# ragoragino/partitionedhashjoin

Measured on AMD Instinct MI355X. Metric: probe+build tuples/sec at 10M⋈200M; achieved HBM GB/s vs roofline, 1/2/4/8 GPU, higher is better.
Workload: dtype int64

## Files before the change

### partitionedhashjoin_amd/csrc/phj_capi.hip

```cpp
#include <hip/hip_runtime.h>

#include <algorithm>
#include <atomic>
#include <cmath>
#include <cstdio>
#include <cstdlib>
#include <cstring>
#include <exception>
#include <functional>
#include <string>
#include <type_traits>
#include <unordered_map>
#include <vector>

#ifndef PHJ_PREAGG
#define PHJ_PREAGG 1
#endif
#ifndef PHJ_HOT_EARLY_R
#define PHJ_HOT_EARLY_R 1
#endif
#ifndef PHJ_HOT_FREE_CUS
#define PHJ_HOT_FREE_CUS 6
#endif
#ifndef PHJ_COL_LOAD16
#define PHJ_COL_LOAD16 0
#endif
#ifndef PHJ_P1_PROF
#define PHJ_P1_PROF 0
#endif
#ifndef PHJ_CL_PROF
#define PHJ_CL_PROF 0
#endif

#include "../../include/phj.h"
#include "phj_cluster.h"
#include "phj_join.h"
#include "phj_inner.h"
#include "phj_outer.h"
#include "phj_index.h"
#include "phj_ordinal.h"
#include "phj_agg.h"
#include "phj_mat.h"
#include "phj_partition.h"
#include "phj_hot.h"
#include "phj_table.h"
#include "phj_member.h"
#include "phj_lookup.h"

using namespace phj;

namespace {

constexpr double kNPDefaultRatio = 2.0;
constexpr uint32_t kNPRegionBuckets = 1024;
constexpr int kOnePassMax = 256;
// ... 126 lines not shown
    DevBuf mat_mark, mat_cnt, mat_rows;
    DevBuf row_hit, row_only, row_cnt;
    DevBuf agg_acc, agg_cnt, agg_rows, agg_res;
    uint64_t agg_n = 0;
    uint64_t mat_n = 0;
    uint64_t idx_n = 0;
    DevBuf gather_bad;
    std::vector<hipEvent_t> evpool;
    size_t evnext = 0;
    std::vector<TimerRec> timers;
    std::string err;
    Tuning tune;
    bool last_fused = false;
    bool dry = false;
    hipEvent_t last_ev = nullptr;
    hipStream_t last_ev_stream = nullptr;
    uint32_t since_ev = 0;
    unsigned long long* count_host = nullptr;
    unsigned long long* count_pin = nullptr;
    unsigned long long* count_pin_dev = nullptr;
    DevBuf cl_done;
    bool count_pin_failed = false, count_pinned = false;
    unsigned long long* split_words = nullptr;
    bool defer_timers = false;
    bool lean_timers = false;
    bool timer_skipped = false;
    void* p1_clear = nullptr;
    size_t p1_clear_bytes = 0;
    void* p1_cleared = nullptr;
    void* s_zeroed = nullptr;
    size_t s_zeroed_bytes = 0;
    void* s_zero_pending = nullptr;
    size_t s_zero_pending_bytes = 0;
    int poison = -1;
    DevBuf hot;
    void* hot_clean = nullptr;
    uint32_t hot_clean_nb = 0;
    int hot_mode = 0;
    bool hot_on = false, hot_ran = false;
    uint64_t hot_n = 0;
    uint32_t hot_min_mass = 0;
    hipEvent_t hot_fork = nullptr, hot_join = nullptr;
    uint32_t p1_free_cus = 0;
    bool p1_cols = false;
    std::vector<phj_index*> indexes;
};

struct phj_index {
    phj_ctx* owner = nullptr;
    IxBucket* tab = nullptr;
    size_t bytes = 0;
    NPHome g{};
    int hk = 0;
    uint64_t seed = 0;
    uint64_t rows = 0, distinct = 0;
    uint32_t max_wgs = 1;
    uint32_t flags = 0;
    int64_t* first_rows = nullptr;
    uint32_t acc_wgs = 1;
};

namespace {

int set_err(phj_ctx* c, int code, const std::string& msg) {
    if (c) c->err = msg;
    return code;
}

#define PHJ_HIP(ctx, expr)                                                                   \
    do {                                                                                     \
        hipError_t e_ = (expr);                                                              \
        if (e_ != hipSuccess)                                                                \
            return set_err(ctx, PHJ_ERR_HIP,                                                 \
                           std::string(#expr) + ": " + hipGetErrorString(e_));               \
    } while (0)

#define PHJ_LAUNCHED(ctx, what)                                                              \
    do {                                                                                     \
        (ctx)->since_ev++;                                                                   \
        hipError_t e_ = hipGetLastError();                                                   \
        if (e_ != hipSuccess)                                                                \
            return set_err(ctx, PHJ_ERR_HIP, std::string("launch ") + what + ": " +         \
                                                 hipGetErrorString(e_));                     \
    } while (0)

#define PHJ_TRY(expr)           \
    do {                        \
        int rc_ = (expr);       \
        if (rc_ != PHJ_OK) return rc_; \
    } while (0)

int ensure(phj_ctx* c, DevBuf& b, size_t bytes) {
    if (bytes == 0) bytes = 16;
    if (b.bytes >= bytes) return PHJ_OK;
    if (b.p) {
        PHJ_HIP(c, hipStreamSynchronize(c->stream));
        PHJ_HIP(c, hipStreamSynchronize(c->aux));
        PHJ_HIP(c, hipFree(b.p));
        b.p = nullptr;
        b.bytes = 0;
    }
    const size_t rounded = (bytes + 4095) & ~size_t(4095);
    hipError_t e = hipMalloc(&b.p, rounded);
    if (e != hipSuccess) {
        b.p = nullptr;
        return set_err(c, PHJ_ERR_NOMEM, "hipMalloc(" + std::to_string(rounded) + "): " + hipGetErrorString(e));
    }
    b.bytes = rounded;
    if (c->poison >= 0) {
        PHJ_HIP(c, hipMemsetAsync(b.p, c->poison, rounded, c->stream));
        PHJ_HIP(c, hipStreamSynchronize(c->stream));
    }
    return PHJ_OK;
}

void free_buf(DevBuf& b) {
    if (b.p) (void)hipFree(b.p);
    b.p = nullptr;
    b.bytes = 0;
}

hipEvent_t new_event() {
    hipEvent_t e = nullptr;
    const unsigned tries[3] = {hipEventDisableSystemFence, hipEventReleaseToDevice, hipEventDefault};
    for (unsigned f : tries) {
        if (hipEventCreateWithFlags(&e, f) == hipSuccess) break;
        (void)hipGetLastError();
        e = nullptr;
    }
    return e;
// ... 340 lines not shown
        size_t l;
        bool operator==(const Key& o) const { return f == o.f && b == o.b && l == o.l; }
    };
    struct Hash {
        size_t operator()(const Key& k) const {
            return std::hash<const void*>()(k.f) ^ (static_cast<size_t>(k.b) << 20) ^ (k.l * 0x9E3779B97F4A7C15ull);
        }
    };
    thread_local std::unordered_map<Key, int, Hash> cache;
    const Key k{kfn, block, lds};
    auto it = cache.find(k);
    if (it != cache.end()) return it->second;
    int occ = 0;
    if (hipOccupancyMaxActiveBlocksPerMultiprocessor(&occ, kfn, block, lds) != hipSuccess) {
        (void)hipGetLastError();
        occ = 0;
    }
    cache.emplace(k, occ);
    return occ;
}

template <int BLOCK, int ITEMS, bool IN_AOS, bool OUT_AOS, int ROWS = 0>
int launch_pass_t(phj_ctx* c, int hk, const PassArgs& a, uint32_t grid, const std::string& prefix,
                  uint64_t n, uint32_t hist_len) {
    static_assert(ROWS == 0 || IN_AOS, "row numbers are synthesised by pass 1");
    if (ROWS != 0 && a.keys_only) return set_err(c, PHJ_ERR_INVALID, "row-number pass 1: no keys-only form");
    constexpr uint64_t kcol = ROWS == 1 ? 8 : 0;
    constexpr int T = BLOCK * ITEMS;
    constexpr int NW = BLOCK / 64;
    const size_t hist_lds = static_cast<size_t>(NW) * a.nbins * 4;
    const size_t sc_lds = scatter_lds_bytes(T, a.nbins, NW, a.chunk_cursor != nullptr);
    const std::string hname = prefix + ".hist", cname = prefix + ".scan", sname = prefix + ".scatter";
    if (a.chunk_cursor) {
        const bool zeroed = a.chunk_cursor == c->s_zeroed && chunk_state_bytes(a.nbins) <= c->s_zeroed_bytes;
        if (a.chunk_cursor == c->s_zeroed) c->s_zeroed = nullptr;
        if (a.chunk_cursor == c->p1_cleared) c->p1_cleared = nullptr;
        else if (!zeroed) PHJ_HIP(c, hipMemsetAsync(a.chunk_cursor, 0, chunk_state_bytes(a.nbins), c->ks));
        c->since_ev++;
        const uint64_t sbytes = n * (a.keys_only ? 24 : 32) - (c->p1_cols ? n * 8 : 0) - n * kcol + (a.out_dig ? n * (a.dig_wide ? 2 : 1) : 0);
        PHJ_TRY(timer_begin(c, sname.c_str(), sbytes));
        if constexpr (IN_AOS && OUT_AOS && ITEMS <= 8) {
            const uint32_t ntiles = static_cast<uint32_t>((n + T - 1) / T);
            const uint32_t per = (ntiles + a.nshards - 1) / a.nshards;
            const bool pipe = a.keys_only && c->tune.p1_pipe && BLOCK == 512 && ITEMS == 8;
            const bool is_r = prefix.rfind("R.", 0) == 0;
            const bool hot = a.hot_code != nullptr;
            const size_t lds = pipe ? chunk_pipe_lds_bytes(T, a.nbins) + chunk_pipe_hot_lds_bytes(a.nbins, hot ? 1 : 0)
                               : a.keys_only ? chunk_codes_lds_bytes(T, a.nbins) : sc_lds;
            const void* kfn = nullptr;
            int kblock = BLOCK;
            bool cols_form = false;
            if (a.keys_only && pipe) {
                if constexpr (BLOCK == 512 && ITEMS == 8) {
                    const int dpt = a.nbins > 2 * BLOCK ? 4 : a.nbins > BLOCK ? 2 : 1;
                    if (c->tune.p1_block == 1024) {
                        kblock = 1024;
                        const int kpf = is_r ? 1 : 2;
                        if (hot && dpt == 4) return set_err(c, PHJ_ERR_STATE, "hot-key pre-aggregation: more digits than threads");
                        if (c->p1_cols && dpt == 4) return set_err(c, PHJ_ERR_STATE, "key column: more digits than threads");
                        const int cols = !c->p1_cols ? 0 : PHJ_COL_LOAD16 != 0 && n >= 2 ? 2 : 1;
                        cols_form = cols != 0;
                        kfn = with_hash(hk, [&](auto h) {
                            constexpr int HK = decltype(h)::value;
                            return dpt == 4 ? pipe1024<HK, 2>(kpf) : pipe1024<HK, 1>(kpf, hot, cols);
                        });
                    } else if (hot) {
                        return set_err(c, PHJ_ERR_STATE, "hot-key pre-aggregation needs the 1024-thread code pass");
                    } else
                        kfn = with_hash(hk, [&](auto h) {
                            constexpr int HK = decltype(h)::value;
                            return dpt == 4 ? reinterpret_cast<const void*>(&k_chunk_codes_pipe<BLOCK, ITEMS, HK, 4>)
                                 : dpt == 2 ? reinterpret_cast<const void*>(&k_chunk_codes_pipe<BLOCK, ITEMS, HK, 2>)
                                            : reinterpret_cast<const void*>(&k_chunk_codes_pipe<BLOCK, ITEMS, HK, 1>);
                        });
                }
            } else if (a.keys_only) {
                if constexpr (BLOCK == 512 && ITEMS == 8) {
                    if (a.nbins > BLOCK)
                        kfn = with_hash(hk, [&](auto h) {
                            constexpr int HK = decltype(h)::value;
                            return a.nbins > 2 * BLOCK ? reinterpret_cast<const void*>(&k_chunk_codes<BLOCK, ITEMS, HK, 4>)
                                                       : reinterpret_cast<const void*>(&k_chunk_codes<BLOCK, ITEMS, HK, 2>);
                        });
                }
                if (!kfn && a.nbins > BLOCK) return set_err(c, PHJ_ERR_INVALID, "keys-only pass 1: more digits than threads");
                if (!kfn)
                    kfn = with_hash(hk, [](auto h) {
                        return reinterpret_cast<const void*>(&k_chunk_codes<BLOCK, ITEMS, decltype(h)::value>);
                    });
            } else
// ... 218 lines not shown
    a.nbits = pl.bits1;
    a.f = digit_fn(pl, 1);
    if (dcol) {
        a.out_dig = S.dig.p;
        a.dig_wide = dbytes == 2 ? 1u : 0u;
        a.dig2_mask = pl.dmask2;
    }
    if (chunked) {
        a.keys_only = ko ? 1u : 0u;
        a.chunk_cursor = static_cast<uint32_t*>(S.ccur.p);
        a.sink = static_cast<unsigned long long*>(S.csink.p);
        a.chunk_tab = static_cast<unsigned long long*>(S.ctab.p);
        a.maxch = maxch;
        a.pool_stride = pool_stride;
        a.nshards = nshards;
        S.ctab_dirty = n > 0;
        S.chunk_check = n > 0;
    }
    unsigned long long* kept = nullptr;
    if (c->hot_on && &S == &c->side[PHJ_SIDE_PROBE]) {
        if (!S.hcoded) return set_err(c, PHJ_ERR_STATE, "hot-key pre-aggregation needs the chunked code pass");
        uint32_t* st = static_cast<uint32_t*>(c->hot.p);
        a.hot_code = reinterpret_cast<const unsigned long long*>(st + kHotCounters);
        a.hot_w = reinterpret_cast<unsigned long long*>(st + kHotCounters) + static_cast<size_t>(pl.nb1) * kHotPer;
        a.hot_ctl = reinterpret_cast<const uint32_t*>(a.hot_w + static_cast<size_t>(pl.nb1) * kHotPer);
        a.hot_min_mass = c->hot_min_mass;
        kept = reinterpret_cast<unsigned long long*>(const_cast<uint32_t*>(a.hot_ctl) + 2);
    }
    uint32_t* tb2 = pl.npass == 2 ? static_cast<uint32_t*>(S.tbase2.p) : nullptr;
    c->p1_cols = cols;
    const int rc1 = launch_pass(c, pl.hk, true, p1_aos, a, nt1, std::string(tag) + ".p1", n, nt1 * pl.nb1, rows);
    c->p1_cols = false;
    PHJ_TRY(rc1);
    if (chunked) {
        uint4* clr = nullptr;
        if (c->p1_clear) {
            clr = static_cast<uint4*>(c->p1_clear);
            c->p1_cleared = c->p1_clear;
            c->p1_clear = nullptr;
        }
        {
            hipLaunchKernelGGL(k_pass1_finish_sizes, dim3(1), dim3(kFinSizesBlock), 0, c->ks, a.chunk_cursor, pl.nb1, nshards, n, tile2,
                               static_cast<uint32_t*>(S.bounds1.p), tb2, zero, clr, static_cast<uint32_t>(c->p1_clear_bytes / 16), kept);
            PHJ_LAUNCHED(c, "k_pass1_finish_sizes");
        }
    } else {
        hipLaunchKernelGGL(k_pass1_finish, dim3(1), dim3(kFinBlock), 0, c->ks, a.hist, nt1, pl.nb1, n,
                           pl.npass == 2 ? tile2 : tile, static_cast<uint32_t*>(S.bounds1.p), tb2);
        PHJ_LAUNCHED(c, "k_pass1_finish");
    }
    if (pl.npass == 1) {
        S.view.keys = static_cast<const int64_t*>(S.kA.p);
        S.view.payloads = static_cast<const int64_t*>(S.pA.p);
        S.view.bounds = static_cast<const uint32_t*>(S.bounds1.p);
    } else {
        PassArgs b{};
        b.in_keys = static_cast<const int64_t*>(S.kA.p);
        b.in_pays = p1_aos ? nullptr : static_cast<const int64_t*>(S.pA.p);
        b.out_keys = static_cast<int64_t*>(S.kB.p);
        b.out_pays = static_cast<int64_t*>(S.pB.p);
        b.hist = static_cast<uint32_t*>(S.hist2.p);
        b.seg_bounds = static_cast<const uint32_t*>(S.bounds1.p);
        b.tile_base = tb2;
        b.tile_seg = static_cast<const uint32_t*>(S.tseg2.p);
        b.nseg = pl.nb1;
        b.keys_only = a.keys_only;
// ... 521 lines not shown
            a.r_bounds[g] = bounds[g];
        }
    }
    a.nseg = static_cast<uint32_t>(nseg);
    a.nb1 = pl.nb1;
    a.cap = static_cast<uint32_t>(c->tune.cl_cap);
    a.lim = cl_lim(a.cap);
    a.e1 = cluster_empty0(pl);
    a.gtab = static_cast<uint64_t*>(c->ht_tab.p);
    a.count = static_cast<unsigned long long*>(c->count.p);
    return a;
}

int cluster_big_fill(phj_ctx* c, const Plan& pl, int nseg, const int64_t* const* codes, const uint32_t* const* bounds,
                     uint64_t nR, SideState* RT = nullptr) {
    if (nseg < 1 || nseg > kHtSegs) return set_err(c, PHJ_ERR_INVALID, "build segments must be in [1,16]");
    const uint64_t slots = 4 * nR + 2ull * pl.nb1;
    if (slots >= (1ull << 32)) return set_err(c, PHJ_ERR_RANGE, "build side too large for 32-bit table slots");
    PHJ_TRY(ensure(c, c->ht_tab, slots * 8));
    PHJ_TRY(ensure(c, c->count, 32));
    if (c->dry) return PHJ_OK;
    ClusterArgs a = cluster_args(c, pl, nseg, codes, bounds, RT);
    hipLaunchKernelGGL(k_cluster_big_fill, dim3(pl.nb1), dim3(256), 0, c->ks, a);
    PHJ_LAUNCHED(c, "k_cluster_big_fill");
    return PHJ_OK;
}

bool count_pin_ready(phj_ctx* c) {
    if (c->count_pin) return true;
    if (c->count_pin_failed) return false;
    void* h = nullptr;
    void* d = nullptr;
    if (hipHostMalloc(&h, 64, hipHostMallocMapped | hipHostMallocCoherent) != hipSuccess ||
        hipHostGetDevicePointer(&d, h, 0) != hipSuccess || ensure(c, c->cl_done, 4) != PHJ_OK ||
        hipMemset(c->cl_done.p, 0, 4) != hipSuccess) {
        (void)hipGetLastError();
        if (h) (void)hipHostFree(h);
        c->count_pin_failed = true;
        return false;
    }
    c->count_pin = static_cast<unsigned long long*>(h);
    c->count_pin_dev = static_cast<unsigned long long*>(d);
    return true;
}

int probe_cluster(phj_ctx* c, const Plan& pl, SideState& PS, int nseg, const int64_t* const* codes,
                  const uint32_t* const* bounds, SideState* RT = nullptr, bool pin = false) {
    if (c->dry || PS.nt2 == 0) return PHJ_OK;
    if (!PS.hcoded) return set_err(c, PHJ_ERR_STATE, "the LDS join needs the keys-only pass 1 (codes)");
    ClusterArgs a = cluster_args(c, pl, nseg, codes, bounds, RT);
    SideState& RS = c->side[PHJ_SIDE_BUILD];
    if (RS.chunk_check) {
        a.err_r = static_cast<const uint32_t*>(RS.ccur.p) + chunk_err_word(RS.plan.nb1);
        RS.chunk_check = false;
    }
    a.s_codes = PS.p2.in_keys;
    a.tile_base = PS.p2.tile_base;
    a.tile_seg = PS.p2.tile_seg;
    a.tile_start = PS.p2.tile_start;
    a.tile_cnt = PS.p2.tile_cnt;
    if (PS.chunk_check) {
        a.err = static_cast<const uint32_t*>(PS.ccur.p) + chunk_err_word(PS.plan.nb1);
        PS.chunk_check = false;
    }
    if (c->tune.timers) {
        a.split = static_cast<unsigned long long*>(c->count.p) + 2;
        c->split_words = a.split;
    }
    constexpr int B = kClBlock, I = kClItems;
    const size_t lds = cluster_lds_bytes(a.cap);
    constexpr bool PR = PHJ_CL_PROF != 0;
    if (PR) {
        PHJ_TRY(ensure(c, c->cl_prof, 64 * 8));
        a.prof = static_cast<unsigned long long*>(c->cl_prof.p);
        PHJ_HIP(c, hipMemsetAsync(a.prof, 0, kClProfWords * 8, c->ks));
    }
    if (c->hot_on && RT && &PS == &c->side[PHJ_SIDE_PROBE]) {
        const uint32_t* st = static_cast<const uint32_t*>(c->hot.p);
        a.hot_code = reinterpret_cast<const unsigned long long*>(st + kHotCounters);
        a.hot_w = a.hot_code + static_cast<size_t>(pl.nb1) * kHotPer;
        a.hot_ctl = reinterpret_cast<const uint32_t*>(a.hot_w + static_cast<size_t>(pl.nb1) * kHotPer);
        a.hot_min_mass = c->hot_min_mass;
    }
    const void* kfn = !RT          ? reinterpret_cast<const void*>(&k_cluster_probe<B, I, 3, true, PR, false>)
                      : a.hot_code ? reinterpret_cast<const void*>(&k_cluster_probe<B, I, 3, true, PR, true, true>)
                                   : reinterpret_cast<const void*>(&k_cluster_probe<B, I, 3, true, PR, true>);
    int per_cu = 0;
    if ((per_cu = occupancy(kfn, B, lds)) < 1) per_cu = 1;
    per_cu = std::max(1, std::min<int>(per_cu, static_cast<int>(160 * 1024 / (lds + 256))));
    const uint32_t want = (PS.nt2 + 7) & ~7u;
    const uint32_t grid = std::max<uint32_t>(8, std::min<uint32_t>(want, static_cast<uint32_t>(per_cu) * c->num_cus) & ~7u);
    void* kargs[] = {&a};
    PHJ_TRY(launch_kernel(c, kfn, dim3(grid), dim3(B), kargs, lds, "k_cluster_probe"));
    if (PR) {
        unsigned long long h[kClProfWords] = {};
        PHJ_HIP(c, hipMemcpyAsync(h, a.prof, sizeof(h), hipMemcpyDeviceToHost, c->ks));
        PHJ_HIP(c, hipStreamSynchronize(c->ks));
        std::fprintf(stderr, "cl_prof grid %u: cold %.1f us, clear+runs %.1f us, inserts %.1f us, prefetch %.1f us; builds %llu, cold %llu\n",
                     grid, h[0] / 100.0, h[1] / 100.0, h[2] / 100.0, h[3] / 100.0, h[4], h[5]);
    }
    a.split = nullptr;
    a.err = nullptr;
    a.err_r = nullptr;
    if (pin && c->tune.count_pin && count_pin_ready(c)) {
        reinterpret_cast<volatile unsigned long long*>(c->count_pin)[1] = ~0ull;
        a.host_out = c->count_pin_dev;
        a.done = static_cast<uint32_t*>(c->cl_done.p);
        c->count_pinned = true;
        a.s_clear = static_cast<uint4*>(PS.ccur.p);
        a.s_clear16 = static_cast<uint32_t>(chunk_state_bytes(PS.plan.nb1) / 16);
        c->s_zero_pending = PS.ccur.p;
        c->s_zero_pending_bytes = chunk_state_bytes(PS.plan.nb1);
    }
    hipLaunchKernelGGL(k_cluster_probe_big, dim3(std::max<uint32_t>(kProbeBigGrid, (pl.nb1 + 255) / 256)), dim3(256), 0, c->ks, a);
    PHJ_LAUNCHED(c, "k_cluster_probe_big");
    return PHJ_OK;
}

int get_count(phj_ctx* c, uint64_t* out, bool pair = false) {
    if (c->count_pinned) {
        c->count_pinned = false;
        const volatile unsigned long long* v = c->count_pin;
        if (c->defer_timers) {
            for (uint32_t i = 1; v[1] == ~0ull; i++) {
                if ((i & 4095u) == 0) {
                    const hipError_t q = hipStreamQuery(c->ks);
                    if (q == hipSuccess) break;
                    if (q != hipErrorNotReady) PHJ_HIP(c, q);
                }
                __builtin_ia32_pause();
            }
            std::atomic_thread_fence(std::memory_order_acquire);
        } else {
            PHJ_HIP(c, hipStreamSynchronize(c->ks));
        }
        const unsigned long long failed = v[1];
        if (failed == 0) {
            c->s_zeroed = c->s_zero_pending;
            c->s_zeroed_bytes = c->s_zero_pending_bytes;
        }
        c->s_zero_pending = nullptr;
        if (failed != ~0ull) {
            *out = v[0];
            if (pair && failed) {
                c->side[PHJ_SIDE_PROBE].chunk_check = true;
                const int rc = check_chunk_errors(c);
                return rc != PHJ_OK ? rc : chunk_table_error(c, 0);
            }
            return check_chunk_errors(c);
        }
    }
    if (!c->count_host && hipHostMalloc(reinterpret_cast<void**>(&c->count_host), 16, hipHostMallocDefault) != hipSuccess) {
        (void)hipGetLastError();
        c->count_host = nullptr;
    }
    unsigned long long h[2] = {0, 0};
    unsigned long long* dst = c->count_host ? c->count_host : h;
    PHJ_HIP(c, hipMemcpyAsync(dst, c->count.p, pair ? 16 : 8, hipMemcpyDeviceToHost, c->ks));
    PHJ_HIP(c, hipStreamSynchronize(c->ks));
    *out = dst[0];
    if (pair && dst[1]) {
        c->side[PHJ_SIDE_PROBE].chunk_check = true;
        const int rc = check_chunk_errors(c);
        return rc != PHJ_OK ? rc : chunk_table_error(c, 0);
    }
    return check_chunk_errors(c);
}

int join_nopart_ct(phj_ctx* c, const phj_join_params* p, phj_join_result* r) {
    SideState& R = c->side[PHJ_SIDE_BUILD];
    SideState& S = c->side[PHJ_SIDE_PROBE];
    uint32_t k = 2;
    while (k < 22 && (R.n >> k) > 300) k++;
    phj_join_params pp = *p;
// ... 2093 lines not shown
            if (rc == PHJ_OK) rc = timer_end(c);
            if (rc == PHJ_OK) rc = phase_mark(&tr);
            c->ks = c->stream;
            return rc;
        };
        if (order == 2) {
            PHJ_TRY(r_chain(t0));
            PHJ_HIP(c, hipStreamWaitEvent(c->stream, tr, 0));
        }
        const bool pre_clear = r_main && !early_r && c->tune.r_chunk && R.n > 0 && !c->dry;
        if (pre_clear) {
            PHJ_TRY(ensure(c, R.ccur, chunk_state_bytes(cpl.nb1)));
            c->p1_clear = R.ccur.p;
            c->p1_clear_bytes = chunk_state_bytes(cpl.nb1);
        }
        if (early_r) {
            for (hipEvent_t* e : {&c->hot_fork, &c->hot_join})
                if (!*e && !(*e = new_event())) return set_err(c, PHJ_ERR_HIP, "hipEventCreate failed");
            PHJ_HIP(c, hipEventRecord(c->hot_fork, c->stream));
        }
        struct HotScope {
            phj_ctx* c;
            bool ok = false;
            ~HotScope() {
                c->hot_on = false;
                if (!ok) c->hot_clean = nullptr;
            }
        } hot_scope{c};
        if (hot) PHJ_TRY(hot_begin(c, cpl, S));
        if (early_r) {
            int rc = r_chain(c->hot_fork);
            if (rc == PHJ_OK && hipEventRecord(c->hot_join, c->aux) != hipSuccess) rc = set_err(c, PHJ_ERR_HIP, "hipEventRecord failed");
            PHJ_TRY(rc);
        }
        const int prc = partition_side(c, PHJ_SIDE_PROBE, cpl, true, static_cast<unsigned long long*>(c->count.p));
        c->p1_clear = nullptr;
        if (prc != PHJ_OK) {
            c->p1_cleared = nullptr;
            return prc;
        }
        if (!S.hcoded) PHJ_HIP(c, hipMemsetAsync(c->count.p, 0, 32, c->stream));
        if (order != 2 && !early_r) {
            const int rc = r_chain(t0);
            c->p1_cleared = nullptr;
            PHJ_TRY(rc);
        }
        if (!r_main) PHJ_HIP(c, hipStreamWaitEvent(c->stream, tr, 0));
        if (early_r) PHJ_HIP(c, hipStreamWaitEvent(c->stream, c->hot_join, 0));
        if (c->hot_on && R.n > 0 && !RT) return set_err(c, PHJ_ERR_STATE, "hot-key pre-aggregation needs R's chunked code pass");
        PHJ_TRY(phase_mark(&t1));
        PHJ_TRY(timer_begin_split(c, R.n * 8, S.n * 8));
        if (c->lean_timers && c->tune.timers) {
            const hipEvent_t e = c->timers.back().a;
            c->timers.insert(c->timers.end() - 2, TimerRec{"build.big", 0, e, e});
        }
        c->count_pinned = false;
        PHJ_TRY(probe_cluster(c, cpl, S, 1, &rcodes, &rbnd, RT, true));
        PHJ_TRY(timer_end_split(c));
        PHJ_TRY(phase_mark(&p1));
        uint64_t m = 0;
        PHJ_TRY(get_count(c, &m, true));
        r->matches = m;
        r->partition_ms = elapsed(c, t0, t1);
        {
            const double t = elapsed(c, t1, p1), fb = c->tune.timers && !c->defer_timers ? fused_build_fraction(c) : 0.0;
            r->build_ms = elapsed(c, b0, tr) + t * fb;
            r->probe_ms = t * (1.0 - fb);
        }
        r->total_ms = elapsed(c, t0, p1);
        r->num_partitions = requested;
        r->algorithmic_bytes = R.n * (24 + 8) + S.n * (24 + 8) - (r_cols ? R.n * 8 : 0) - (s_cols ? S.n * 8 : 0);
        hot_scope.ok = true;
        return fill_timers(c, r);
    }
    PHJ_TRY(need_tuples_both(c, false, "phj_join"));
    refine_plan(c, pl, R.n);
    if (use_p2probe(c, pl, S.n, R.n)) {
        PHJ_TRY(ensure(c, c->count, 32));
        PHJ_TRY(mark(c, &t0));
        PHJ_TRY(partition_side(c, PHJ_SIDE_PROBE, pl, true, static_cast<unsigned long long*>(c->count.p)));
        PHJ_HIP(c, hipStreamWaitEvent(c->aux, t0, 0));
// ... 556 lines not shown
```

### partitionedhashjoin_amd/csrc/phj_cluster.h

```cpp
#pragma once

#include <hip/hip_runtime.h>
#include <stdint.h>

#include "phj_hash.h"
#include "phj_partition.h"
#include "phj_table.h"

namespace phj {

constexpr int kClBlock = 1024, kClItems = 4;
constexpr uint32_t kClCapMax = 16384;
constexpr uint32_t kClCpl = kClCapMax * 3 / 4 / kClBlock;

__host__ __device__ __forceinline__ uint32_t cl_lim(uint32_t cap) { return cap / 4 * 3; }

__host__ __device__ __forceinline__ uint32_t cl_big_cap(uint32_t m) { return ht_cap_for(m + (m + 1) / 2); }

struct ClusterArgs {
    const int64_t* s_codes;
    const uint32_t* tile_base;
    const uint32_t* tile_seg;
    const uint32_t* tile_start;
    const uint32_t* tile_cnt;
    const int64_t* r_codes[kHtSegs];
    const uint32_t* r_bounds[kHtSegs];
    uint32_t nseg, nb1;
    uint32_t cap, lim;
    uint64_t e1;
    uint64_t* gtab;
    unsigned long long* count;
    const uint32_t* err;
    unsigned long long* split;
    unsigned long long* prof;
    const uint32_t* rt_base;
    const uint32_t* rt_start;
    const uint32_t* rt_cnt;
    const int64_t* r_pool;
    const uint32_t* err_r;
    unsigned long long* host_out;
    uint32_t* done;
    uint4* s_clear;
    uint32_t s_clear16;
    const unsigned long long* hot_code;
    const unsigned long long* hot_w;
    const uint32_t* hot_ctl;
    uint32_t hot_min_mass;
};

__device__ __forceinline__ bool cl_hot_live(const ClusterArgs& a) {
    return a.hot_code && a.hot_ctl[kHotCtlEntries] != 0 && a.hot_ctl[kHotCtlMass] >= a.hot_min_mass;
}

__device__ __forceinline__ bool cl_big(uint32_t m, uint32_t runs, uint32_t lim) { return m > lim || runs > kHtSegs; }
constexpr int kClProfWords = 6;

template <int TM = -1, bool HOT = false>
__device__ __forceinline__ void cl_runs(const ClusterArgs& a, uint32_t d, uint32_t* sseg, const int64_t** sptr,
                                        uint32_t* sB, uint32_t* sM, uint32_t* sN, unsigned long long* shot = nullptr,
                                        const unsigned long long* const* hotp = nullptr) {
    const uint32_t tid = threadIdx.x;
    if (TM == 1 || (TM == -1 && a.rt_base)) {
        if (HOT && tid - 64u < 2 * kHotPer) {
            const uint32_t j = tid - 64u;
            shot[j] = (*hotp)[d * kHotPer + (j < kHotPer ? j : a.nb1 * kHotPer + j - kHotPer)];
        }
        if (tid < 64) {
            const uint32_t t0 = a.rt_base[d], nt = a.rt_base[d + 1] - t0;
            uint32_t lo = 0, len = 0;
            if (tid < nt && nt <= static_cast<uint32_t>(kHtSegs)) {
                lo = a.rt_start[t0 + tid];
                len = a.rt_cnt[t0 + tid];
            }
            uint32_t x = len;
#pragma unroll
            for (int o = 1; o < kHtSegs; o <<= 1) {
                const uint32_t y = __shfl_up(x, o, 64);
                if (tid >= static_cast<uint32_t>(o)) x += y;
            }
            if (tid < nt && nt <= static_cast<uint32_t>(kHtSegs)) {
                sseg[tid + 1] = x;
                sptr[tid] = a.r_pool + lo - (x - len);
            }
            if (tid == 0) {
                sseg[0] = 0;
                const uint32_t b0 = a.r_bounds[0][d];
                *sB = b0;
                *sM = a.r_bounds[0][d + 1] - b0;
                *sN = nt;
            }
        }
        return;
    }
    if (tid < 64) {
        uint32_t lo = 0, len = 0;
        if (tid < a.nseg) {
            lo = a.r_bounds[tid][d];
            len = a.r_bounds[tid][d + 1] - lo;
        }
        uint32_t x = len;
#pragma unroll
        for (int o = 1; o < kHtSegs; o <<= 1) {
            const uint32_t y = __shfl_up(x, o, 64);
            if (tid >= static_cast<uint32_t>(o)) x += y;
        }
        uint32_t b = lo;
#pragma unroll
        for (int o = 1; o < kHtSegs; o <<= 1) b += __shfl_xor(b, o, 64);
        if (tid < a.nseg) {
            sseg[tid + 1] = x;
            sptr[tid] = a.r_codes[tid] + lo - (x - len);
        }
        if (tid == 0) {
            sseg[0] = 0;
            *sB = b;
        }
        if (tid == a.nseg - 1) *sM = x;
        if (tid == 0) *sN = a.nseg;
    }
}

__device__ __forceinline__ uint32_t cl_seg_of(const uint32_t* sseg, uint32_t nseg, uint32_t r) {
    uint32_t g = 0;
#pragma unroll
    for (uint32_t step = kHtSegs / 2; step >= 1; step >>= 1)
        if (g + step < nseg && sseg[g + step] <= r) g += step;
    return g;
}

__global__ __launch_bounds__(256) void k_cluster_big_fill(ClusterArgs a) {
    __shared__ uint32_t sseg[kHtSegs + 1];
    __shared__ const int64_t* sptr[kHtSegs];
    __shared__ uint32_t sB, sM, sN;
    const uint32_t d = blockIdx.x, tid = threadIdx.x;
    cl_runs(a, d, sseg, sptr, &sB, &sM, &sN);
    __syncthreads();
    const uint32_t m = sM;
    if (!cl_big(m, sN, a.lim)) return;
    const uint64_t e = d == 0 ? a.e1 : 0ull;
    const uint32_t cap = cl_big_cap(m);
    uint64_t* t = a.gtab + 4ull * sB + 2ull * d;
    for (uint32_t sl = tid; sl < cap; sl += 256) t[sl] = e;
    __threadfence();
    __syncthreads();
    if (a.rt_base) {
        for (uint32_t ti = a.rt_base[d]; ti < a.rt_base[d + 1]; ti++) {
            const int64_t* src = a.r_pool + a.rt_start[ti];
            const uint32_t c = a.rt_cnt[ti];
            for (uint32_t r = tid; r < c; r += 256) ht_insert(t, cap / 2 - 1, e, static_cast<uint64_t>(src[r]));
        }
        return;
    }
    for (uint32_t r = tid; r < m; r += 256) {
        const uint32_t g = cl_seg_of(sseg, a.nseg, r);
        ht_insert(t, cap / 2 - 1, e, static_cast<uint64_t>(sptr[g][r]));
    }
}

__device__ __forceinline__ bool cl_is_big(const ClusterArgs& a, uint32_t d) {
    if (a.rt_base) return cl_big(a.r_bounds[0][d + 1] - a.r_bounds[0][d], a.rt_base[d + 1] - a.rt_base[d], a.lim);
    uint32_t m = 0;
    for (uint32_t g = 0; g < a.nseg; g++) m += a.r_bounds[g][d + 1] - a.r_bounds[g][d];
    return cl_big(m, a.nseg, a.lim);
}

constexpr uint32_t kProbeBigGrid = 64;
__global__ __launch_bounds__(256) void k_cluster_probe_big(ClusterArgs a) {
    __shared__ uint32_t sseg[kHtSegs + 1];
    __shared__ const int64_t* sptr[kHtSegs];
    __shared__ uint32_t sB, sM, sN;
    __shared__ uint32_t red[4];
    __shared__ uint32_t list[256], nlist;
    __shared__ uint32_t hlist[256], nhlist, met[kHotPer];
    const uint32_t tid = threadIdx.x, G = gridDim.x;
    if (tid == 0) nlist = nhlist = 0;
    __syncthreads();
    const bool hot = a.rt_base && cl_hot_live(a);
    for (uint32_t d = blockIdx.x + tid * G; d < a.nb1; d += 256 * G) {
        if (cl_is_big(a, d)) {
            list[atomicAdd(&nlist, 1u)] = d;
        } else if (hot && a.tile_base[d] == a.tile_base[d + 1]) {
            bool any = false;
#pragma unroll
            for (uint32_t k = 0; k < kHotPer; k++) any = any || a.hot_w[static_cast<size_t>(d) * kHotPer + k] != 0;
            if (any) hlist[atomicAdd(&nhlist, 1u)] = d;
        }
    }
    __syncthreads();
    const uint32_t nbig = nlist, nhot = nhlist;
    uint32_t hits = 0;
    unsigned long long hsum = 0;
    for (uint32_t k = 0; k < nbig; k++) {
        const uint32_t d = list[k];
        cl_runs(a, d, sseg, sptr, &sB, &sM, &sN);
        __syncthreads();
        const uint64_t e = d == 0 ? a.e1 : 0ull;
        const uint32_t bmask = cl_big_cap(sM) / 2 - 1;
        const ulonglong2* g2 = reinterpret_cast<const ulonglong2*>(a.gtab + 4ull * sB + 2ull * d);
        __syncthreads();
        for (uint32_t t = a.tile_base[d]; t < a.tile_base[d + 1]; t++) {
            const uint32_t lo = a.tile_start[t], c = a.tile_cnt[t];
            for (uint32_t i = tid; i < c; i += 256) {
                const uint64_t cc = static_cast<uint64_t>(a.s_codes[lo + i]);
                uint32_t b = static_cast<uint32_t>(cc >> kHtBucketShift) & bmask;
                for (;;) {
                    const ulonglong2 w = g2[b];
                    if (w.x == cc || w.y == cc) {
                        hits++;
                        break;
                    }
                    if (w.y == e) break;
                    b = (b + 1) & bmask;
                }
            }
        }
        if (hot && tid < kHotPer) {
            const uint64_t cc = a.hot_code[static_cast<size_t>(d) * kHotPer + tid];
            const unsigned long long wt = a.hot_w[static_cast<size_t>(d) * kHotPer + tid];
// ... 36 lines not shown
#pragma unroll
                for (uint32_t u = 0; u < U; u++) {
                    if (r0 + u * 64 + l >= c) continue;
#pragma unroll
                    for (uint32_t q = 0; q < kHotPer; q++)
                        if (v[u] == hc[q] && hw[q] != 0) met[q] = 1;
                }
            }
        }
        __syncthreads();
        if (tid < kHotPer && met[tid]) hsum += a.hot_w[static_cast<size_t>(d) * kHotPer + tid];
        __syncthreads();
    }
    if (nbig == 0 && nhot == 0 && !a.host_out) return;
    __shared__ uint32_t clear_state;
    if (hsum) {
        atomicAdd(a.count, hsum);
        __threadfence();
    }
    uint32_t x = hits;
#pragma unroll
    for (int o = 32; o > 0; o >>= 1) x += __shfl_down(x, o, 64);
    if ((tid & 63) == 0) red[tid >> 6] = x;
    __syncthreads();
    if (tid == 0) {
        clear_state = 0;
        const unsigned long long s = static_cast<unsigned long long>(red[0]) + red[1] + red[2] + red[3];
        if (s) atomicAdd(a.count, s);
        if (a.host_out) {
            __threadfence();
            if (atomicAdd(a.done, 1u) == G - 1) {
                __threadfence();
                const unsigned long long c0 = atomicAdd(a.count, 0ull), c1 = atomicAdd(a.count + 1, 0ull);
                a.host_out[0] = c0;
                __threadfence_system();
                a.host_out[1] = c1;
                __threadfence_system();
                atomicExch(a.done, 0u);
                clear_state = a.s_clear && c1 == 0 ? 1u : 0u;
            }
        }
    }
    __syncthreads();
    if (clear_state)
        for (uint32_t i = tid; i < a.s_clear16; i += 256) a.s_clear[i] = make_uint4(0, 0, 0, 0);
}

__host__ __device__ constexpr size_t cluster_lds_bytes(uint32_t cap) { return static_cast<size_t>(cap) * 9; }
#ifndef PHJ_CL_ASM
#define PHJ_CL_ASM 1
#endif
template <int BLOCK, int ITEMS, int PF = 1, bool PRE = true, bool PROF = false, bool TM = false, bool HOTR = false,
          bool ASMW = PHJ_CL_ASM != 0>
__global__ __launch_bounds__(BLOCK) void k_cluster_probe(ClusterArgs a) {
    static_assert(!HOTR || TM, "the hot entries are staged with a cluster's R tiles");
    constexpr int CPL = kClCapMax * 3 / 4 / BLOCK;
    extern __shared__ __attribute__((aligned(16))) uint64_t tab[];
    uint32_t* const fill = reinterpret_cast<uint32_t*>(tab + a.cap);
    __shared__ uint32_t sseg_[2][kHtSegs + 1];
    __shared__ const int64_t* sptr_[2][kHtSegs];
    __shared__ uint32_t sB_[2], sM_[2], sN_[2];
    __shared__ unsigned long long shot_[2][HOTR ? 2 * kHotPer : 1], shsum;
    __shared__ const unsigned long long* shotp;
    __shared__ uint32_t shctl[2];
    __shared__ uint32_t red[BLOCK / 64];
    constexpr uint32_t MR = 512;
    __shared__ uint32_t smeta[3][MR];
    const uint32_t tid = threadIdx.x, wave = tid >> 6, lane = tid & 63;
    const uint32_t total = a.tile_base[a.nb1];
    const uint32_t G = gridDim.x, r8 = (blockIdx.x & 7u) * (G >> 3) + (blockIdx.x >> 3);
    const uint32_t t_lo = static_cast<uint32_t>(static_cast<uint64_t>(total) * r8 / G);
    const uint32_t t_hi = static_cast<uint32_t>(static_cast<uint64_t>(total) * (r8 + 1) / G);
    uint32_t hits = 0;
    const unsigned long long clk0 = wall_clock64();
    unsigned long long clk_b = 0;
    __shared__ unsigned long long prof[PROF ? kClProfWords : 1];
    if (PROF && tid < kClProfWords) prof[tid] = 0;
    if (t_lo < t_hi) {
        typedef long long v2i __attribute__((ext_vector_type(2)));
        v2i kv[PF][ITEMS / 2];
        uint32_t vm[PF], dq[PF];
        uint32_t mbase = 0xffffffffu;
        auto stage = [&](uint32_t base) {
            __syncthreads();
            for (uint32_t i = tid; i < MR; i += BLOCK) {
                const uint32_t ti = min(base + i, t_hi - 1);
                smeta[0][i] = a.tile_seg[ti];
                smeta[1][i] = a.tile_start[ti];
                smeta[2][i] = a.tile_cnt[ti];
            }
            __builtin_amdgcn_s_waitcnt(0xF70);
            __syncthreads();
            mbase = base;
        };
        auto load = [&](uint32_t t, v2i* k, uint32_t& m, uint32_t& dd) {
            if (t - mbase >= MR && t < t_hi) stage(t);
            const uint32_t j = min(t, t_hi - 1) - mbase;
            dd = smeta[0][j];
            const uint32_t lo = smeta[1][j];
            const uint32_t c = t < t_hi ? smeta[2][j] : 0u;
            m = 0;
            const v2i* src = reinterpret_cast<const v2i*>(a.s_codes + lo);
            const uint32_t last = c ? (c - 1) / 2 : 0u;
#pragma unroll
            for (int i = 0; i < ITEMS; i += 2) {
// ... 194 lines not shown
        while (more) {
#pragma unroll
            for (int f = 0; f < PF; f++) {
                more = step(f);
                if (!more) break;
            }
        }
        if constexpr (ASMW) {
#pragma unroll
            for (int f = 0; f < PF; f++) __asm__ volatile("s_waitcnt vmcnt(0)" : "+v"(kv[f][0]), "+v"(kv[f][1]));
        }
    }
    uint32_t x = hits;
#pragma unroll
    for (int o = 32; o > 0; o >>= 1) x += __shfl_down(x, o, 64);
    if (lane == 0) red[wave] = x;
    __syncthreads();
    if (tid == 0) {
        unsigned long long s = 0;
        for (int w = 0; w < BLOCK / 64; w++) s += red[w];
        if constexpr (HOTR)
            if (t_lo < t_hi) s += shsum;
        if (s) atomicAdd(a.count, s);
        if (a.split) {
            const unsigned long long all = wall_clock64() - clk0;
            atomicAdd(&a.split[0], clk_b);
            atomicAdd(&a.split[1], all - clk_b);
        }
        if (PROF && a.prof)
            for (int w = 0; w < kClProfWords; w++) atomicAdd(&a.prof[w], prof[PROF ? w : 0]);
    }
    fold_pass1_error(a.err, a.count);
    fold_pass1_error(a.err_r, a.count);
}

}
```

Measured before the change: 192.6 billion.

## Add early count publish, R cursor tail-clear, snapped probe ranges, earlier join wait

Bundles several changes. The R-side chunk-cursor state is now zeroed by the tail probe kernel, so the next call skips a memset. R's code pass uses prefetch depth 2 when free CUs exist. The hot-join event wait moves to right after pass 1. Probe blocks snap their tile ranges to cluster boundaries. The last cluster-probe block publishes the count to pinned host memory early when no big or hot-tileless clusters exist, and the big-cluster kernel then skips its scan. These cut memsets, stream-wait latency and host readback latency, at the cost of extra scans of tile_base in every block plus added ticket/flag state.

```diff
diff --git a/partitionedhashjoin_amd/csrc/phj_capi.hip b/partitionedhashjoin_amd/csrc/phj_capi.hip
--- a/partitionedhashjoin_amd/csrc/phj_capi.hip
+++ b/partitionedhashjoin_amd/csrc/phj_capi.hip
@@ -21,6 +21,15 @@
 #endif
 #ifndef PHJ_HOT_FREE_CUS
 #define PHJ_HOT_FREE_CUS 6
+#endif
+#ifndef PHJ_R_TAILCLEAR
+#define PHJ_R_TAILCLEAR 1
+#endif
+#ifndef PHJ_R_KPF2
+#define PHJ_R_KPF2 1
+#endif
+#ifndef PHJ_JOINWAIT_EARLY
+#define PHJ_JOINWAIT_EARLY 1
 #endif
 #ifndef PHJ_COL_LOAD16
 #define PHJ_COL_LOAD16 0
@@ -213,6 +222,11 @@
     size_t s_zeroed_bytes = 0;
     void* s_zero_pending = nullptr;
     size_t s_zero_pending_bytes = 0;
+    void* r_zeroed = nullptr;
+    size_t r_zeroed_bytes = 0;
+    void* r_zero_pending = nullptr;
+    size_t r_zero_pending_bytes = 0;
+    hipEvent_t wait_after_p1 = nullptr;
     int poison = -1;
     DevBuf hot;
     void* hot_clean = nullptr;
@@ -277,6 +291,8 @@
     if (b.p) {
         PHJ_HIP(c, hipStreamSynchronize(c->stream));
         PHJ_HIP(c, hipStreamSynchronize(c->aux));
+        for (void** z : {&c->s_zeroed, &c->s_zero_pending, &c->r_zeroed, &c->r_zero_pending})
+            if (*z == b.p) *z = nullptr;
         PHJ_HIP(c, hipFree(b.p));
         b.p = nullptr;
         b.bytes = 0;
@@ -683,8 +699,10 @@
     const size_t sc_lds = scatter_lds_bytes(T, a.nbins, NW, a.chunk_cursor != nullptr);
     const std::string hname = prefix + ".hist", cname = prefix + ".scan", sname = prefix + ".scatter";
     if (a.chunk_cursor) {
-        const bool zeroed = a.chunk_cursor == c->s_zeroed && chunk_state_bytes(a.nbins) <= c->s_zeroed_bytes;
+        const bool zeroed = (a.chunk_cursor == c->s_zeroed && chunk_state_bytes(a.nbins) <= c->s_zeroed_bytes) ||
+                            (a.chunk_cursor == c->r_zeroed && chunk_state_bytes(a.nbins) == c->r_zeroed_bytes);
         if (a.chunk_cursor == c->s_zeroed) c->s_zeroed = nullptr;
+        if (a.chunk_cursor == c->r_zeroed) c->r_zeroed = nullptr;
         if (a.chunk_cursor == c->p1_cleared) c->p1_cleared = nullptr;
         else if (!zeroed) PHJ_HIP(c, hipMemsetAsync(a.chunk_cursor, 0, chunk_state_bytes(a.nbins), c->ks));
         c->since_ev++;
@@ -706,7 +724,8 @@
                     const int dpt = a.nbins > 2 * BLOCK ? 4 : a.nbins > BLOCK ? 2 : 1;
                     if (c->tune.p1_block == 1024) {
                         kblock = 1024;
-                        const int kpf = is_r ? 1 : 2;
+                        const bool r_kpf2 = PHJ_R_KPF2 != 0 && PHJ_P1_PROF == 0 && c->p1_free_cus > 0;
+                        const int kpf = is_r && !r_kpf2 ? 1 : 2;
                         if (hot && dpt == 4) return set_err(c, PHJ_ERR_STATE, "hot-key pre-aggregation: more digits than threads");
                         if (c->p1_cols && dpt == 4) return set_err(c, PHJ_ERR_STATE, "key column: more digits than threads");
                         const int cols = !c->p1_cols ? 0 : PHJ_COL_LOAD16 != 0 && n >= 2 ? 2 : 1;
@@ -991,6 +1010,11 @@
     const int rc1 = launch_pass(c, pl.hk, true, p1_aos, a, nt1, std::string(tag) + ".p1", n, nt1 * pl.nb1, rows);
     c->p1_cols = false;
     PHJ_TRY(rc1);
+    if (chunked && c->wait_after_p1) {
+        const hipEvent_t e = c->wait_after_p1;
+        c->wait_after_p1 = nullptr;
+        PHJ_HIP(c, hipStreamWaitEvent(c->ks, e, 0));
+    }
     if (chunked) {
         uint4* clr = nullptr;
         if (c->p1_clear) {
@@ -1578,8 +1602,8 @@
     void* h = nullptr;
     void* d = nullptr;
     if (hipHostMalloc(&h, 64, hipHostMallocMapped | hipHostMallocCoherent) != hipSuccess ||
-        hipHostGetDevicePointer(&d, h, 0) != hipSuccess || ensure(c, c->cl_done, 4) != PHJ_OK ||
-        hipMemset(c->cl_done.p, 0, 4) != hipSuccess) {
+        hipHostGetDevicePointer(&d, h, 0) != hipSuccess || ensure(c, c->cl_done, 16) != PHJ_OK ||
+        hipMemset(c->cl_done.p, 0, 16) != hipSuccess) {
         (void)hipGetLastError();
         if (h) (void)hipHostFree(h);
         c->count_pin_failed = true;
@@ -1636,8 +1660,19 @@
     per_cu = std::max(1, std::min<int>(per_cu, static_cast<int>(160 * 1024 / (lds + 256))));
     const uint32_t want = (PS.nt2 + 7) & ~7u;
     const uint32_t grid = std::max<uint32_t>(8, std::min<uint32_t>(want, static_cast<uint32_t>(per_cu) * c->num_cus) & ~7u);
+    const bool pinned = pin && c->tune.count_pin && count_pin_ready(c);
+    if (pinned) {
+        reinterpret_cast<volatile unsigned long long*>(c->count_pin)[1] = ~0ull;
+        if (PHJ_CL_EARLYCOUNT != 0) {
+            a.early_out = c->count_pin_dev;
+            a.ticket = static_cast<uint32_t*>(c->cl_done.p) + 1;
+            a.early = static_cast<uint32_t*>(c->cl_done.p) + 2;
+        }
+    }
     void* kargs[] = {&a};
     PHJ_TRY(launch_kernel(c, kfn, dim3(grid), dim3(B), kargs, lds, "k_cluster_probe"));
+    a.early_out = nullptr;
+    a.ticket = nullptr;
     if (PR) {
         unsigned long long h[kClProfWords] = {};
         PHJ_HIP(c, hipMemcpyAsync(h, a.prof, sizeof(h), hipMemcpyDeviceToHost, c->ks));
@@ -1648,8 +1683,7 @@
     a.split = nullptr;
     a.err = nullptr;
     a.err_r = nullptr;
-    if (pin && c->tune.count_pin && count_pin_ready(c)) {
-        reinterpret_cast<volatile unsigned long long*>(c->count_pin)[1] = ~0ull;
+    if (pinned) {
         a.host_out = c->count_pin_dev;
         a.done = static_cast<uint32_t*>(c->cl_done.p);
         c->count_pinned = true;
@@ -1657,6 +1691,13 @@
         a.s_clear16 = static_cast<uint32_t>(chunk_state_bytes(PS.plan.nb1) / 16);
         c->s_zero_pending = PS.ccur.p;
         c->s_zero_pending_bytes = chunk_state_bytes(PS.plan.nb1);
+        c->r_zero_pending = nullptr;
+        if (PHJ_R_TAILCLEAR != 0 && RT && RT->ccur.p) {
+            a.r_clear = static_cast<uint4*>(RT->ccur.p);
+            a.r_clear16 = static_cast<uint32_t>(chunk_state_bytes(RT->plan.nb1) / 16);
+            c->r_zero_pending = RT->ccur.p;
+            c->r_zero_pending_bytes = chunk_state_bytes(RT->plan.nb1);
+        }
     }
     hipLaunchKernelGGL(k_cluster_probe_big, dim3(std::max<uint32_t>(kProbeBigGrid, (pl.nb1 + 255) / 256)), dim3(256), 0, c->ks, a);
     PHJ_LAUNCHED(c, "k_cluster_probe_big");
@@ -1684,8 +1725,11 @@
         if (failed == 0) {
             c->s_zeroed = c->s_zero_pending;
             c->s_zeroed_bytes = c->s_zero_pending_bytes;
+            c->r_zeroed = c->r_zero_pending;
+            c->r_zeroed_bytes = c->r_zero_pending_bytes;
         }
         c->s_zero_pending = nullptr;
+        c->r_zero_pending = nullptr;
         if (failed != ~0ull) {
             *out = v[0];
             if (pair && failed) {
@@ -3845,8 +3889,11 @@
             int rc = r_chain(c->hot_fork);
             if (rc == PHJ_OK && hipEventRecord(c->hot_join, c->aux) != hipSuccess) rc = set_err(c, PHJ_ERR_HIP, "hipEventRecord failed");
             PHJ_TRY(rc);
+            if (PHJ_JOINWAIT_EARLY != 0) c->wait_after_p1 = c->hot_join;
         }
         const int prc = partition_side(c, PHJ_SIDE_PROBE, cpl, true, static_cast<unsigned long long*>(c->count.p));
+        const bool join_waited = early_r && PHJ_JOINWAIT_EARLY != 0 && !c->wait_after_p1;
+        c->wait_after_p1 = nullptr;
         c->p1_clear = nullptr;
         if (prc != PHJ_OK) {
             c->p1_cleared = nullptr;
@@ -3859,7 +3906,7 @@
             PHJ_TRY(rc);
         }
         if (!r_main) PHJ_HIP(c, hipStreamWaitEvent(c->stream, tr, 0));
-        if (early_r) PHJ_HIP(c, hipStreamWaitEvent(c->stream, c->hot_join, 0));
+        if (early_r && !join_waited) PHJ_HIP(c, hipStreamWaitEvent(c->stream, c->hot_join, 0));
         if (c->hot_on && R.n > 0 && !RT) return set_err(c, PHJ_ERR_STATE, "hot-key pre-aggregation needs R's chunked code pass");
         PHJ_TRY(phase_mark(&t1));
         PHJ_TRY(timer_begin_split(c, R.n * 8, S.n * 8));
diff --git a/partitionedhashjoin_amd/csrc/phj_cluster.h b/partitionedhashjoin_amd/csrc/phj_cluster.h
--- a/partitionedhashjoin_amd/csrc/phj_cluster.h
+++ b/partitionedhashjoin_amd/csrc/phj_cluster.h
@@ -42,6 +42,11 @@
     uint32_t* done;
     uint4* s_clear;
     uint32_t s_clear16;
+    uint4* r_clear;
+    uint32_t r_clear16;
+    unsigned long long* early_out;
+    uint32_t* ticket;
+    uint32_t* early;
     const unsigned long long* hot_code;
     const unsigned long long* hot_w;
     const uint32_t* hot_ctl;
@@ -94,9 +99,11 @@
     }
     if (tid < 64) {
         uint32_t lo = 0, len = 0;
+        uint32_t g = tid;
+        __asm__ volatile("" : "+v"(g));
         if (tid < a.nseg) {
-            lo = a.r_bounds[tid][d];
-            len = a.r_bounds[tid][d + 1] - lo;
+            lo = a.r_bounds[g][d];
+            len = a.r_bounds[g][d + 1] - lo;
         }
         uint32_t x = len;
 #pragma unroll
@@ -109,7 +116,7 @@
         for (int o = 1; o < kHtSegs; o <<= 1) b += __shfl_xor(b, o, 64);
         if (tid < a.nseg) {
             sseg[tid + 1] = x;
-            sptr[tid] = a.r_codes[tid] + lo - (x - len);
+            sptr[tid] = a.r_codes[g] + lo - (x - len);
         }
         if (tid == 0) {
             sseg[0] = 0;
@@ -164,6 +171,14 @@
     return cl_big(m, a.nseg, a.lim);
 }
 
+__device__ __forceinline__ bool cl_tileless_hot(const ClusterArgs& a, uint32_t d) {
+    if (a.tile_base[d] != a.tile_base[d + 1]) return false;
+    bool any = false;
+#pragma unroll
+    for (uint32_t k = 0; k < kHotPer; k++) any = any || a.hot_w[static_cast<size_t>(d) * kHotPer + k] != 0;
+    return any;
+}
+
 constexpr uint32_t kProbeBigGrid = 64;
 __global__ __launch_bounds__(256) void k_cluster_probe_big(ClusterArgs a) {
     __shared__ uint32_t sseg[kHtSegs + 1];
@@ -173,17 +188,19 @@
     __shared__ uint32_t list[256], nlist;
     __shared__ uint32_t hlist[256], nhlist, met[kHotPer];
     const uint32_t tid = threadIdx.x, G = gridDim.x;
-    if (tid == 0) nlist = nhlist = 0;
+    __shared__ uint32_t early_;
+    if (tid == 0) {
+        nlist = nhlist = 0;
+        early_ = a.early && a.host_out ? __hip_atomic_load(a.early, __ATOMIC_RELAXED, __HIP_MEMORY_SCOPE_AGENT) : 0u;
+    }
     __syncthreads();
+    const bool early = early_ != 0;
     const bool hot = a.rt_base && cl_hot_live(a);
-    for (uint32_t d = blockIdx.x + tid * G; d < a.nb1; d += 256 * G) {
+    for (uint32_t d = blockIdx.x + tid * G; d < a.nb1 && !early; d += 256 * G) {
         if (cl_is_big(a, d)) {
             list[atomicAdd(&nlist, 1u)] = d;
-        } else if (hot && a.tile_base[d] == a.tile_base[d + 1]) {
-            bool any = false;
-#pragma unroll
-            for (uint32_t k = 0; k < kHotPer; k++) any = any || a.hot_w[static_cast<size_t>(d) * kHotPer + k] != 0;
-            if (any) hlist[atomicAdd(&nhlist, 1u)] = d;
+        } else if (hot && cl_tileless_hot(a, d)) {
+            hlist[atomicAdd(&nhlist, 1u)] = d;
         }
     }
     __syncthreads();
@@ -286,23 +303,36 @@
             if (atomicAdd(a.done, 1u) == G - 1) {
                 __threadfence();
                 const unsigned long long c0 = atomicAdd(a.count, 0ull), c1 = atomicAdd(a.count + 1, 0ull);
-                a.host_out[0] = c0;
-                __threadfence_system();
-                a.host_out[1] = c1;
-                __threadfence_system();
+                if (!early) {
+                    a.host_out[0] = c0;
+                    __threadfence_system();
+                    a.host_out[1] = c1;
+                    __threadfence_system();
+                } else {
+                    atomicExch(a.early, 0u);
+                }
                 atomicExch(a.done, 0u);
                 clear_state = a.s_clear && c1 == 0 ? 1u : 0u;
             }
         }
     }
     __syncthreads();
-    if (clear_state)
+    if (clear_state) {
         for (uint32_t i = tid; i < a.s_clear16; i += 256) a.s_clear[i] = make_uint4(0, 0, 0, 0);
+        for (uint32_t i = tid; i < a.r_clear16; i += 256) a.r_clear[i] = make_uint4(0, 0, 0, 0);
+    }
 }
 
 __host__ __device__ constexpr size_t cluster_lds_bytes(uint32_t cap) { return static_cast<size_t>(cap) * 9; }
 #ifndef PHJ_CL_ASM
 #define PHJ_CL_ASM 1
+#endif
+#ifndef PHJ_CL_SNAP
+#define PHJ_CL_SNAP 1
+#endif
+constexpr uint32_t kClSnapTau = 5;
+#ifndef PHJ_CL_EARLYCOUNT
+#define PHJ_CL_EARLYCOUNT 1
 #endif
 template <int BLOCK, int ITEMS, int PF = 1, bool PRE = true, bool PROF = false, bool TM = false, bool HOTR = false,
           bool ASMW = PHJ_CL_ASM != 0>
@@ -323,8 +353,22 @@
     const uint32_t tid = threadIdx.x, wave = tid >> 6, lane = tid & 63;
     const uint32_t total = a.tile_base[a.nb1];
     const uint32_t G = gridDim.x, r8 = (blockIdx.x & 7u) * (G >> 3) + (blockIdx.x >> 3);
-    const uint32_t t_lo = static_cast<uint32_t>(static_cast<uint64_t>(total) * r8 / G);
-    const uint32_t t_hi = static_cast<uint32_t>(static_cast<uint64_t>(total) * (r8 + 1) / G);
+    uint32_t t_lo = static_cast<uint32_t>(static_cast<uint64_t>(total) * r8 / G);
+    uint32_t t_hi = static_cast<uint32_t>(static_cast<uint64_t>(total) * (r8 + 1) / G);
+    if constexpr (PHJ_CL_SNAP != 0) {
+        __shared__ uint32_t snap_[2];
+        if (tid < 2) snap_[tid] = 0;
+        __syncthreads();
+        for (uint32_t d = 1 + tid; d < a.nb1; d += BLOCK) {
+            const uint32_t s = a.tile_base[d];
+            if (s + kClSnapTau >= t_lo && s <= t_lo + kClSnapTau) atomicMax(&snap_[0], s + 1);
+            if (s + kClSnapTau >= t_hi && s <= t_hi + kClSnapTau) atomicMax(&snap_[1], s + 1);
+        }
+        __syncthreads();
+        const uint32_t s_lo = __builtin_amdgcn_readfirstlane(snap_[0]), s_hi = __builtin_amdgcn_readfirstlane(snap_[1]);
+        if (r8 != 0 && s_lo) t_lo = s_lo - 1;
+        if (r8 + 1 != G && s_hi) t_hi = s_hi - 1;
+    }
     uint32_t hits = 0;
     const unsigned long long clk0 = wall_clock64();
     unsigned long long clk_b = 0;
@@ -585,6 +629,35 @@
     }
     fold_pass1_error(a.err, a.count);
     fold_pass1_error(a.err_r, a.count);
-}
-
-}
+    if constexpr (PHJ_CL_EARLYCOUNT != 0) {
+        if (!a.early_out) return;
+        __shared__ uint32_t last_, found_;
+        if (tid == 0) {
+            found_ = 0;
+            __threadfence();
+            last_ = atomicAdd(a.ticket, 1u) == G - 1 ? 1u : 0u;
+        }
+        __syncthreads();
+        if (!last_) return;
+        const bool hot = a.rt_base && cl_hot_live(a);
+        bool found = false;
+        for (uint32_t d = tid; d < a.nb1; d += BLOCK) found = found || cl_is_big(a, d) || (hot && cl_tileless_hot(a, d));
+        if (found) found_ = 1;
+        __syncthreads();
+        if (tid == 0) {
+            const bool none = found_ == 0;
+            if (none) {
+                __threadfence();
+                const unsigned long long c0 = atomicAdd(a.count, 0ull), c1 = atomicAdd(a.count + 1, 0ull);
+                a.early_out[0] = c0;
+                __threadfence_system();
+                a.early_out[1] = c1;
+                __threadfence_system();
+            }
+            atomicExch(a.ticket, 0u);
+            atomicExch(a.early, none ? 1u : 0u);
+        }
+    }
+}
+
+}
```

After: 185.1 billion. 0.961x the previous value.
